# ekimb/rust-mdbg

Measured on AMD Instinct MI355X. Metric: Gbases/s ingested to k-min-mer graph, higher is better.
Workload: dtype u64

## Files before the change

### rust_mdbg_amd/csrc/context.inc

```
namespace {
struct KeptReads {
    void* blk = nullptr; size_t cap = 0; void* xblk = nullptr; size_t xcap = 0;
    u64 n_reads = 0, n_bases = 0, n_words = 0, n_exc = 0;
    KeptReads() = default; KeptReads(const KeptReads&) = delete; KeptReads& operator=(const KeptReads&) = delete;
    ~KeptReads() { if (blk) mdbg_block_free(blk, cap); if (xblk) mdbg_block_free(xblk, xcap); }
    uint2* planes() const { return (uint2*)blk; }
    u64* offsets() const { return (u64*)blk + n_words; }
    u64* exc_pos() const { return (u64*)xblk; }
    u8* exc_val() const { return (u8*)xblk + n_exc * 8; }
    u64 bytes() const { return n_words * 8 + (n_reads + 1) * 8 + n_exc * 9; }
};
struct Batch { u64 first_ordinal; u32 n_reads; u32 slot0; u64 m0, m1; u64 owned = ~0ull;
               u64 list_off = ~0ull;
               bool mread_ok = true;
               u32 src_rank = ~0u;
               u64 n_bases = 0;
               bool partial = false;
               u64 adm_word = ~0ull;
               std::shared_ptr<KeptReads> kept; };

enum { SH_DISTINCT = 0, SH_OWNED, SH_OWNINS, SH_FIN_WRAPPED, SH_FIN_DISTINCT, N_SHARD_ARRAYS };
enum { SC_CARRY = 0, SC_NDISTINCT, SC_NWINDOWS, SC_FIN0, SC_FIN1, SC_FIN2, SC_SLOWCOUNT , SC_ERRFLAG , SC_CAPERR , SC_SLOWTOTAL, SC_BATCHWIN, SC_IMPORTERR, SC_PROBEERR , SC_OWNINS, SC_OVERMAX , SC_TOTFIRST, SC_TOTSOLID, SC_SLICEFAIL, SC_DONE , SC_N };

}
// ... 5 lines not shown
    std::mutex err_mu;
    Stage stage[2]; std::mutex stage_mu; std::condition_variable stage_cv;
    mdbg_params P{};
    int dev = 0; hipStream_t stream = nullptr; std::string err; int poisoned = 0;
    u64 scal_seq = 0; bool batchwin_zero = false;
    u64* h_scal = nullptr;
    u64 bound = 0; DevBuf d_t4;
    DevBuf mh, mpos, mread, roff; u64 M = 0; u64 mcap = 0; u32 n_slots = 0;
    u64 slot_end_m = 0;
    u64 pending_m = 0;
    std::vector<Batch> batches; size_t batches_inserted = 0;
    u64 h_known = 0;
    DevBuf bread, tile_recs, slab, n_valid, n_scan, last_read, tile_base, scan_tmp, gran_sum, tile_flags, scalars, phase_dbg, shards;
    u32 slab_cap_min = 0;
    DevBuf tab, mx; u64 cap = 0;
    DevBuf pf_cells, pf_adm;
    u64 pf_n_cells = 0;
    size_t pf_counted = 0;
    bool pf_stale = false, pf_dirty = false;
    u64 n_windows_admitted = 0;
    DevBuf arena, route_out, route_tmp, route_h, route_f; u64 n_records = 0; bool routed = false;
    DevBuf by_maps;
    DevBuf link_ctr;
    DevBuf claim;
    bool claims_ok = false;
    size_t claims_fin_batches = 0; u64 claims_fin_top = 0;
    DevBuf bm_first, bm_solid, pre_first, pre_solid, popc_tmp, bt_dev, fin_out, solid_list, fin_order;
    DevBuf bm_local, pre_local, pre_local2;
    std::vector<u64> so_hash, so_pos, so_off;
    std::vector<u32> q_counts; std::vector<u64> q_off; DevBuf q_dev;
// ... 35 lines not shown
#define HIPCHK(c, call) do { hipError_t e_ = (call); if (e_ != hipSuccess) return fail_hip((c), #call, e_); } while (0)
#define MDBG_ENTER(c, args_ok) if (!(c) || !(args_ok)) return MDBG_E_PARAM; MDBG_LOCK(c); (void)hipSetDevice((c)->dev); if ((c)->poisoned) return fail((c), MDBG_E_STATE, "context is in an error state")
struct HandOver {
    mdbg_ctx* c; const char* what; bool to_host; int err = MDBG_OK;
    template <class T> void col(const T* dev, size_t n, HostRaw<T>& h, const T** dst) {
        if (err) return;
        if (!to_host) { *dst = dev; return; }
        if (!h.resize(n)) { err = fail(c, MDBG_E_NOMEM, what); return; }
        if (n) { const hipError_t e = hipMemcpy(h.data(), dev, n * sizeof(T), hipMemcpyDeviceToHost); if (e != hipSuccess) { err = fail_hip(c, what, e); return; } }
        *dst = h.data();
    }
};
bool nothing_resident(const mdbg_ctx* c) { return c->cap == 0 || c->M == 0; }

u64* scal(mdbg_ctx* c) { return c->scalars.as<u64>(); }
int read_scalars(mdbg_ctx* c, u64* host, bool with_fin = false, bool zero_batchwin = false) {
    if (!c->h_scal) { HIPCHK(c, hipHostMalloc((void**)&c->h_scal, (SC_N + 1) * 8, hipHostMallocMapped)); c->h_scal[SC_N] = 0; }
    const u64 seq = ++c->scal_seq;
    PublishArgs pa{};
    pa.shards[0] = c->shards.as<u64>() + SH_DISTINCT * CTR_SHARDS; pa.idx[0] = SC_NDISTINCT; pa.n_arrays = 1;
    pa.zero_mask = 0; pa.zero_arrays = 0;
    if (with_fin) {
        pa.shards[1] = c->shards.as<u64>() + SH_FIN_WRAPPED * CTR_SHARDS; pa.idx[1] = SC_FIN1; pa.shards[2] = c->shards.as<u64>() + SH_FIN_DISTINCT * CTR_SHARDS; pa.idx[2] = SC_FIN2; pa.n_arrays = 3;
        pa.zero_mask = (1ull << SC_FIN0) | (1ull << SC_FIN1) | (1ull << SC_FIN2); pa.zero_arrays = 0x6u;
    }
    pa.scalars = scal(c); pa.n = SC_N; pa.host = c->h_scal; pa.seq = seq; pa.zero_idx = zero_batchwin ? (u32)SC_BATCHWIN : (u32)SC_N;
    c->batchwin_zero = zero_batchwin;
    launch_publish_scalars(pa, c->stream);
    volatile u64* const flag = c->h_scal + SC_N;
    bool seen = false;
    const double t0 = now_ms();
    for (u32 spins = 0; !seen; ++spins) {
// ... 48 lines not shown
    const u64 mul = owner_bin_mul(c);
    if (!mul || c->batches.empty()) return MDBG_OK;
    Batch& b = which == ~(size_t)0 ? c->batches.back() : c->batches[which];
    fill_mread_of(c, b);
    launch_owner_bins(c->mh.as<u64>(), c->mread.as<u32>(), c->roff.as<u64>(), b.m0, b.m1, c->P.k, mul, d_hist, c->stream);
    return MDBG_OK;
}
int owner_set_table(mdbg_ctx* c, u32 world, const u8* tab) {
    const u64 mul = owner_bin_mul(c);
    if (!mul || !owner_thr(c, world)) return MDBG_OK;
    HIPCHK(c, hipMemcpyAsync(c->own_thr.as<u64>() + OWNER_TAB_AT, tab, OWNER_BINS, hipMemcpyHostToDevice, c->stream));
    HIPCHK(c, hipMemcpyAsync(c->own_thr.as<u64>(), &mul, 8, hipMemcpyHostToDevice, c->stream));
    HIPCHK(c, hipStreamSynchronize(c->stream));
    return MDBG_OK;
}
TableArgs table_args(mdbg_ctx* c) {
    TableArgs T;
    T.tab = c->tab.as<Slot>(); T.cap = c->cap; T.mx = c->mx.as<u64>(); T.A = cascade_of(c->P.min_abundance);
    T.n_distinct = c->shards.as<u64>() + SH_DISTINCT * CTR_SHARDS;
    T.ks.mh = c->mh.as<u64>(); T.ks.arena = c->arena.as<u64>(); T.ks.k = c->P.k;
    T.own_world = c->own_world; T.own_rank = c->own_rank; T.own_thr = owner_thr(c, c->own_world);
    T.probe_err = (u32*)(scal(c) + SC_PROBEERR); T.own_inserted = c->shards.as<u64>() + SH_OWNINS * CTR_SHARDS;
    T.claim = (!c->routed && c->claims_ok) ? c->claim.as<u8>() : nullptr;
    static const bool no_chain = getenv("MDBG_NO_CHAIN") != nullptr;
    T.no_chain = no_chain ? 1u : 0u;
    static const bool weak_fp = getenv("MDBG_WEAK_FP") != nullptr;
    T.fp_mask = weak_fp ? 0x3ull : 0x3FFFFFFFull;
    static const bool count_links = getenv("MDBG_COUNT_LINKS") != nullptr;
    T.link_ctr = nullptr;
    if (count_links) {
        if (!c->link_ctr.p && c->link_ctr.ensure(8, 0, c->stream) == hipSuccess) (void)hipMemsetAsync(c->link_ctr.p, 0, 8, c->stream);
// ... 7 lines not shown
int table_reserve(mdbg_ctx* c, u64 incoming) {
    u64 need = slots_for(c->n_distinct + incoming);
    const u32 A = cascade_of(c->P.min_abundance);
    if (c->cap == 0) {
        u64 want = need;
        if (c->P.table_capacity_hint) want = std::max(want, slots_for(c->P.table_capacity_hint));
        HIPCHK(c, c->tab.ensure(want * sizeof(Slot), 0, c->stream));
        if (A > 2) HIPCHK(c, c->mx.ensure(want * (A - 2) * 8, 0, c->stream));
        c->cap = want;
        launch_clear_table(c->tab.as<Slot>(), c->cap, c->mx.as<u64>(), A > 2 ? c->cap * (A - 2) : 0, c->stream);
        c->claims_ok = !c->routed && c->claim.p != nullptr;
        c->claims_fin_batches = 0;
        return MDBG_OK;
    }
    if (need <= c->cap) return MDBG_OK;
    need = std::max(need, 2 * c->cap);
    DevBuf ntab, nmx;
    HIPCHK(c, ntab.ensure(need * sizeof(Slot), 0, c->stream));
    if (A > 2) HIPCHK(c, nmx.ensure(need * (A - 2) * 8, 0, c->stream));
    launch_clear_table(ntab.as<Slot>(), need, nmx.as<u64>(), A > 2 ? need * (A - 2) : 0, c->stream);
    TableArgs T = table_args(c);
    T.tab = ntab.as<Slot>(); T.cap = need; T.mx = nmx.as<u64>();
    launch_rehash(c->tab.as<Slot>(), c->cap, c->mx.as<u64>(), T, c->stream);
    HIPCHK(c, hipStreamSynchronize(c->stream));
    std::swap(c->tab.p, ntab.p); std::swap(c->tab.cap, ntab.cap);
    std::swap(c->mx.p, nmx.p); std::swap(c->mx.cap, nmx.cap);
    c->cap = need;
    return MDBG_OK;
}

int clear_table(mdbg_ctx* c) {
    c->res.invalidate(FROM_NODES);
    ZeroList z{};
    z.p[0] = c->shards.as<u64>() + SH_DISTINCT * CTR_SHARDS; z.n[0] = CTR_SHARDS; z.p[1] = scal(c) + SC_NDISTINCT; z.n[1] = 2;
    z.p[2] = scal(c) + SC_IMPORTERR; z.n[2] = 1; z.p[3] = scal(c) + SC_PROBEERR; z.n[3] = 1;
    if (c->cap) launch_clear_table(c->tab.as<Slot>(), c->cap, c->mx.as<u64>(), cascade_of(c->P.min_abundance) > 2 ? c->cap * (cascade_of(c->P.min_abundance) - 2) : 0, c->stream, &z);
    else launch_zero_regions(z, c->stream);
    c->n_distinct = 0; c->n_windows = 0; c->n_windows_admitted = 0; c->batches_inserted = 0; c->n_records = 0; c->routed = false;
    c->claims_ok = c->claim.p != nullptr; c->claims_fin_batches = 0;
    return MDBG_OK;
}

#define STAGE_EVENT(c, ev, s) do { if ((c)->timing >= 2) HIPCHK((c), hipEventRecord((ev), (s))); } while (0)
hipEvent_t next_tile_event(mdbg_ctx* c) {
    if (c->timing < 1) return nullptr;
    if (c->tile_ev_used == c->tile_ev.size()) { hipEvent_t e = nullptr; if (hipEventCreate(&e) != hipSuccess) return nullptr; c->tile_ev.push_back(e); }
    return c->tile_ev[c->tile_ev_used++];
}
void collect_tile_events(mdbg_ctx* c) {
    for (size_t i = 0; i + 1 < c->tile_ev_used; i += 2) {
        float ms = 0;
// ... 110 lines not shown
```

### rust_mdbg_amd/csrc/dev_util.hip

```cpp
#include "mdbg_dev.h"
struct ZeroList { u64* p[6]; u64 n[6]; u64* set_p; u64 set_v; };
__global__ __launch_bounds__(256) void zero_regions_kernel(ZeroList z) {
    const u64 i0 = (u64)blockIdx.x * blockDim.x + threadIdx.x, stride = (u64)gridDim.x * blockDim.x;
#pragma unroll
    for (int r = 0; r < 6; ++r) for (u64 i = i0; i < z.n[r]; i += stride) z.p[r][i] = 0;
    if (i0 == 0 && z.set_p) *z.set_p = z.set_v;
}
void launch_zero_regions(const ZeroList& z, hipStream_t s) {
    u64 mx = 1;
    for (int r = 0; r < 6; ++r) mx = z.n[r] > mx ? z.n[r] : mx;
    const unsigned blocks = (unsigned)std::min<u64>(1024, (mx + 255) / 256);
    hipLaunchKernelGGL(zero_regions_kernel, dim3(blocks), dim3(256), 0, s, z);
}
__global__ __launch_bounds__(256) void fill_u64_kernel(u64* __restrict__ p, u64 n, u64 v) {
    for (u64 i = (u64)blockIdx.x * blockDim.x + threadIdx.x; i < n; i += (u64)gridDim.x * blockDim.x) p[i] = v;
}
void launch_fill_u64(u64* p, u64 n, u64 v, hipStream_t s) {
    if (n) hipLaunchKernelGGL(fill_u64_kernel, dim3((unsigned)std::min<u64>(1024, (n + 255) / 256)), dim3(256), 0, s, p, n, v);
}

__global__ __launch_bounds__(256) void sum_shards_kernel(const u64* __restrict__ shards, u64* __restrict__ out) {
    __shared__ u64 ws[4];
    const u64* s = shards + (size_t)blockIdx.x * CTR_SHARDS;
    u64 v = 0;
// ... 66 lines not shown
```

### rust_mdbg_amd/csrc/finalize_api.inc

```
static int fin_setup(mdbg_ctx* c, FinArgs& F, u64& n_words_out, bool byte_maps = false) {
    hipStream_t s = c->stream;
    c->res.invalidate(FROM_NODES);
    F.ath_override = nullptr;
    const u32 k = c->P.k;
        std::vector<Batch> bs = c->batches;
        std::sort(bs.begin(), bs.end(), [](const Batch& a, const Batch& b) { return a.first_ordinal < b.first_ordinal; });
        const u32 nb = (u32)bs.size();
        for (u32 i = 0; i + 1 < nb; ++i)
            if (bs[i].n_reads && bs[i].first_ordinal + bs[i].n_reads > bs[i + 1].first_ordinal) {
                char buf[200]; snprintf(buf, sizeof buf, "read ordinals of two batches overlap: [%llu, +%u) and [%llu, +%u) (first_read_ordinal must be the position of the batch's first record in the whole input)",
                                        (unsigned long long)bs[i].first_ordinal, bs[i].n_reads, (unsigned long long)bs[i + 1].first_ordinal, bs[i + 1].n_reads);
                return fail(c, MDBG_E_PARAM, buf);
            }
        std::vector<u64> fo(nb), rb(nb); std::vector<u32> nr(nb), s0(nb);
        u64 acc = 0;
        for (u32 i = 0; i < nb; ++i) { fo[i] = bs[i].first_ordinal; nr[i] = bs[i].n_reads; s0[i] = bs[i].slot0; rb[i] = acc; acc += bs[i].m1 - bs[i].m0; }
        std::vector<Batch> bs2 = c->batches;
        std::sort(bs2.begin(), bs2.end(), [](const Batch& a, const Batch& b) { return a.slot0 < b.slot0; });
        std::vector<u64> f2(nb), m2(nb), r2(nb); std::vector<u32> s2(nb);
        for (u32 i = 0; i < nb; ++i) { f2[i] = bs2[i].first_ordinal; s2[i] = bs2[i].slot0; }
        {
            std::vector<u32> ord(nb);
            for (u32 i = 0; i < nb; ++i) ord[i] = i;
            std::sort(ord.begin(), ord.end(), [&](u32 a, u32 b) { return bs[a].m0 != bs[b].m0 ? bs[a].m0 < bs[b].m0 : bs[a].m1 < bs[b].m1; });
// ... 279 lines not shown
```

### rust_mdbg_amd/csrc/import_api.inc

```
int mdbg_set_partition(mdbg_ctx* c, uint32_t world, uint32_t rank) {
    if (!c) return MDBG_E_PARAM;
    MDBG_LOCK(c);
    if (world < 1 || world > 4096 || rank >= world) return fail(c, MDBG_E_PARAM, "bad partition");
    if (world > 1 && prefilter_on(c)) return fail(c, MDBG_E_STATE, PF_UNAVAILABLE);
    if (c->n_distinct || c->batches_inserted) return fail(c, MDBG_E_STATE, "set the partition before inserting");
    c->own_world = world; c->own_rank = rank;
    return MDBG_OK;
}

int mdbg_sketch_view(mdbg_ctx* c, mdbg_sketch_store* out) {
    if (!c || !out) return MDBG_E_PARAM;
    MDBG_LOCK(c);
    (void)hipSetDevice(c->dev);
    HIPCHK(c, hipStreamSynchronize(c->stream));
    out->n_minimizers = c->M; out->n_reads = c->n_slots;
    out->d_hashes = c->mh.as<u64>(); out->d_positions = c->mpos.as<u32>(); out->d_read_offsets = c->roff.as<u64>();
    return MDBG_OK;
}

int mdbg_ingest_sketch(mdbg_ctx* c, const uint64_t* d_hashes, const uint32_t* d_positions, const uint64_t* d_read_offsets, uint64_t n_reads,
                       uint64_t first_read_ordinal) {
    if (!c) return MDBG_E_PARAM;
    MDBG_LOCK(c);
    (void)hipSetDevice(c->dev);
// ... 48 lines not shown
}

static int sketch_commit_impl(mdbg_ctx* c, uint64_t region, uint64_t n_minimizers, const uint64_t* d_read_offsets, uint64_t n_reads, uint64_t first_read_ordinal,
                              uint64_t owned_windows, bool with_read_map) {
    MDBG_LOCK(c);
    (void)hipSetDevice(c->dev);
    if (c->poisoned) return fail(c, MDBG_E_STATE, "context is in an error state");
    if (n_minimizers > c->pending_m || region + n_minimizers > c->M) return fail(c, MDBG_E_PARAM, "not a reserved region");
    if (n_reads && !d_read_offsets) return fail(c, MDBG_E_PARAM, "null offsets");
    if (first_read_ordinal + n_reads >= (1ull << (64 - WIN_BITS))) return fail(c, MDBG_E_CAPACITY, "read ordinal too large");
    store_commit_region(c, n_minimizers);
    if (!n_reads) return MDBG_OK;
    hipStream_t s = c->stream;
    u32 slot0 = 0;
    { int e = next_slot0(c, region, n_reads, &slot0); if (e) return e; }
    launch_rebase_offsets_checked(d_read_offsets, (u32)n_reads, region, n_minimizers, c->roff.as<u64>() + slot0, scal(c) + SC_IMPORTERR, s);
    if (with_read_map) launch_fill_mread(c->roff.as<u64>(), slot0, (u32)n_reads, c->mread.as<u32>(), s);
    Batch b; b.first_ordinal = first_read_ordinal; b.n_reads = (u32)n_reads; b.slot0 = slot0; b.m0 = region; b.m1 = region + n_minimizers;
    b.owned = owned_windows; b.mread_ok = with_read_map;
    store_append(c, b);
    return MDBG_OK;
}
int mdbg_sketch_commit(mdbg_ctx* c, uint64_t region, uint64_t n_minimizers, const uint64_t* d_read_offsets, uint64_t n_reads, uint64_t first_read_ordinal,
                       uint64_t owned_windows) {
    if (!c) return MDBG_E_PARAM;
    return sketch_commit_impl(c, region, n_minimizers, d_read_offsets, n_reads, first_read_ordinal, owned_windows, true);
}

int mdbg_owner_counts(mdbg_ctx* c, uint32_t world, uint64_t* counts) {
    if (!c || !counts) return MDBG_E_PARAM;
// ... 136 lines not shown
```

### rust_mdbg_amd/csrc/ingest_api.inc

```
namespace {
constexpr u64 SLAB_BUDGET = 6ull << 30;
int insert_resident_impl(mdbg_ctx* c, bool allow_pending = false);

constexpr const char* TABLE_FULL = "the table filled up during insertion";
int close_round(mdbg_ctx* c, const u64* sc, const char* probe_msg, float ms) {
    if ((u32)sc[SC_PROBEERR]) return fail(c, MDBG_E_PARAM, probe_msg);
    c->ms_insert += ms;
    c->n_windows += sc[SC_BATCHWIN];
    c->n_distinct = sc[SC_NDISTINCT];
    if (sc[SC_IMPORTERR]) return fail(c, MDBG_E_PARAM, "read offsets of an imported sketch are not consistent with its size");
    if ((u32)sc[SC_CAPERR]) return fail(c, MDBG_E_CAPACITY, "a read has more than 2^26 minimizers");
    return MDBG_OK;
}

struct SketchCall {
    const SketchInput& in; const u64* d_offsets; u64 n_reads, n_bases, first_ordinal, n_tiles_total; u32 slot0; bool phase_dbg;
};
int check_sketch_call(mdbg_ctx* c, const SketchInput& in, const u64* d_offsets, u64 n_reads, u64 n_bases, u64 first_ordinal, u64 n_tiles_total) {
    if (in.fmt == FMT_ASCII && !in.d_bases && n_bases) return fail(c, MDBG_E_PARAM, "null bases");
    if (in.fmt == FMT_PLANES && !in.d_planes && n_bases) return fail(c, MDBG_E_PARAM, "null packed words");
    if (!d_offsets) return fail(c, MDBG_E_PARAM, "null offsets");
    if ((((uintptr_t)in.d_bases) | ((uintptr_t)in.d_planes)) & 15) return fail(c, MDBG_E_PARAM, "device bases pointer must be 16-byte aligned");
    if (in.n_exc && (!in.d_exc_pos || !in.d_exc_val)) return fail(c, MDBG_E_PARAM, "null exception list");
    if (in.n_exc >= 0xFFFFFFF0ull) return fail(c, MDBG_E_CAPACITY, "too many exceptions");
// ... 46 lines not shown
    (void)hipStreamSynchronize(s);
    (void)hipMemcpy(h.data(), A.dbg, h.size() * 8, hipMemcpyDeviceToHost);
    double ph[7] = {0, 0, 0, 0, 0, 0, 0}, nc = 0, nv = 0; u64 nfast = 0;
    for (u32 t = 0; t < A.n_tiles; ++t) {
        const u64* q = &h[(size_t)t * 16];
        if (!q[7]) continue;
        ++nfast;
        ph[0] += (double)(q[1] - q[0]); ph[1] += (double)(q[2] - q[1]); ph[2] += (double)(q[3] - q[2]); ph[3] += (double)(q[4] - q[3]);
        ph[4] += (double)(q[5] - q[4]); ph[5] += (double)(q[7] - q[5]);
        nc += (double)q[9]; nv += (double)q[10];
    }
    const double n = nfast ? (double)nfast : 1.0;
    fprintf(stderr, "[mdbg phase timing] tiles=%u fast=%llu avg cycles: load=%.0f compact=%.0f hash=%.0f exact=%.0f rank=%.0f write=%.0f ; candidates=%.1f valid=%.1f slab_cap=%u\n",
            A.n_tiles, (unsigned long long)nfast, ph[0] / n, ph[1] / n, ph[2] / n, ph[3] / n, ph[4] / n, ph[5] / n, nc / n, nv / n, slab_cap);
}
int launch_tiles(mdbg_ctx* c, const SketchCall& k, SketchArgs& A, SketchInit init0, const TileParts& tp, const SlabPlan& sp) {
    hipStream_t s = c->stream;
    const SketchInput& in = k.in;
    A.bread = c->bread.as<u32>(); A.recs = c->tile_recs.as<TileRec>(); A.n_tiles = (u32)k.n_tiles_total;
    A.slab = c->slab.as<Rec>(); A.slab_cap = sp.slab_cap; A.n_valid = c->n_valid.as<u32>(); A.n_scan = c->n_scan.as<u32>(); A.last_read = c->last_read.as<u32>(); A.over_max = (u32*)(scal(c) + SC_OVERMAX);
    A.t4 = c->d_t4.as<u64>();
    A.tile_flags = in.n_exc ? c->tile_flags.as<u8>() : nullptr;
    A.err_flag = (u32*)(scal(c) + SC_ERRFLAG); A.slow_total = (unsigned long long*)(scal(c) + SC_SLOWTOTAL);
    A.read_base = k.slot0; A.bound = c->bound; A.btop = (u32)(c->bound >> (64 - BS_B)); A.force_slow = ((c->P.flags & 1u) || c->P.l > (u32)BS_MAX_L) ? 1u : 0u;
    A.dbg = nullptr;
    { const char* sp_ = getenv("MDBG_STOP_PHASE"); A.stop_phase = sp_ ? (u32)atoi(sp_) : 0u; }
    if (k.phase_dbg) { HIPCHK(c, c->phase_dbg.ensure((size_t)k.n_tiles_total * 128, 0, s)); HIPCHK(c, hipMemsetAsync(c->phase_dbg.p, 0, (size_t)k.n_tiles_total * 128, s)); A.dbg = c->phase_dbg.as<u64>(); }
    const u32 n_gran = (u32)((tp.max_part + SCAN_GRAN - 1) / SCAN_GRAN);
    HIPCHK(c, c->gran_sum.ensure((size_t)n_gran * 8 + 64, 0, s));
    A.block_sum = (unsigned long long*)c->gran_sum.as<u64>();
    init0.zero_arr = c->gran_sum.as<u64>(); init0.zero_arr_n = n_gran;
// ... 2 lines not shown
        HIPCHK(c, hipMemsetAsync(c->tile_flags.p, 0, k.n_tiles_total, s));
        launch_tile_flags(in.d_exc_pos, (u32)in.n_exc, A.n_tiles, c->tile_flags.as<u8>(), s);
    }
    if (c->P.scheme == MDBG_SCHEME_SYNCMERS) {
        A.scheme = 1; A.s = c->P.syncmer_s; A.btop = 0;
        const double v = c->P.density * (double)(1ull << (2 * c->P.l));
        A.bound = !(v > 0.0) ? 0 : (v >= 18446744073709551616.0 ? ~0ull : (u64)v);
        A.force_slow = ((c->P.flags & 1u) || c->P.syncmer_s > 13) ? 1u : 0u;
    }
    u64 t0 = 0;
    for (size_t pi = 0; pi < tp.part_end.size(); ++pi) {
        const u32 nt = (u32)(tp.part_end[pi] - t0);
        Rec* const part_slab = c->slab.as<Rec>();
        A.tile0 = (u32)t0; A.slab = part_slab;
        if (pi) HIPCHK(c, hipMemsetAsync(c->gran_sum.p, 0, (size_t)n_gran * 8, s));
        { hipEvent_t tb = next_tile_event(c), te = next_tile_event(c); launch_sketch(A, nt, s, tb, te); }
        GatherArgs G = gather_args(c, k, (u32)t0, nt, part_slab, sp.slab_cap, A.n_valid, pi + 1 == tp.part_end.size(), sp.gather_tiles);
        G.n_scan = A.n_scan; G.last_read = A.last_read;
        launch_gather(G, c->scan_tmp.as<u64>(), c->tile_base.as<u64>(), scal(c) + SC_CARRY, s, c->gran_sum.as<u64>());
        c->n_tile_launches += 1;
        t0 = tp.part_end[pi];
    }
    c->n_tile_bases += k.n_bases;
    if (k.phase_dbg) dump_phase_timing(A, sp.slab_cap, s);
    return MDBG_OK;
}
int alphabet_rule_pass(mdbg_ctx* c, const SketchArgs& A, u64 first_ordinal) {
    hipStream_t s = c->stream;
    u64 which = ~0ull;
    HIPCHK(c, hipMemcpyAsync(scal(c) + SC_SLOWTOTAL, &which, 8, hipMemcpyHostToDevice, s));
    launch_alphabet_rule(A, (unsigned long long*)(scal(c) + SC_SLOWTOTAL), s);
// ... 17 lines not shown
    L.mh = c->mh.as<u64>(); L.mpos = c->mpos.as<u32>(); L.mread = c->mread.as<u32>(); L.m0 = c->M; L.m1 = m_new;
    L.offsets = k.d_offsets; L.slot0 = k.slot0; L.l = c->P.l; L.hpc = c->P.reads_already_hpc == 0 ? 1u : 0u;
    L.slab = c->slab.as<Rec>(); L.n_valid = c->n_valid.as<u32>();
    launch_lmer_filter(L, in.fmt, in.d_bases, in.d_planes, in.d_exc_pos, in.d_exc_val, (u32)in.n_exc, s);
    HIPCHK(c, hipMemcpyAsync(scal(c) + SC_CARRY, init, 8, hipMemcpyHostToDevice, s));
    const GatherArgs G = gather_args(c, k, 0, nb, L.slab, 256, L.n_valid, true, 1);
    launch_gather(G, c->scan_tmp.as<u64>(), c->tile_base.as<u64>(), scal(c) + SC_CARRY, s);
    u64 sc[SC_N];
    int e = read_scalars(c, sc); if (e) return e;
    m_new = sc[SC_CARRY];
    return MDBG_OK;
}
int launch_fused_insert(mdbg_ctx* c, const SketchCall& k) {
    hipStream_t s = c->stream;
    u32* const ins_flags = (u32*)(scal(c) + SC_CAPERR);
    launch_count_reserve(c->roff.as<u64>(), k.slot0, (u32)k.n_reads, c->P.k, scal(c) + SC_BATCHWIN, (u32*)(scal(c) + SC_DONE), c->shards.as<u64>() + SH_DISTINCT * CTR_SHARDS, scal(c) + SC_NDISTINCT,
                         c->cap, ins_flags + 1, scal(c) + SC_CARRY, c->mcap, (const u32*)(scal(c) + SC_OVERMAX), s);
    if (!c->ev3) HIPCHK(c, hipEventCreate(&c->ev3));
    launch_insert_windows(table_args(c), c->mh.as<u64>(), c->mread.as<u32>(), c->roff.as<u64>(), c->M, c->mcap, k.slot0, k.first_ordinal, scal(c) + SC_NWINDOWS, ins_flags, s, scal(c) + SC_CARRY);
    STAGE_EVENT(c, c->ev3, s);
    return MDBG_OK;
}
int fused_tail(mdbg_ctx* c, const u64* sc, bool* inserted) {
    c->res.invalidate(FROM_NODES);
    if (sc[SC_CAPERR] >> 32) return MDBG_OK;
    c->batches_inserted = c->batches.size();
    *inserted = true;
    float ms = 0;
    if (c->timing >= 2 && hipEventElapsedTime(&ms, c->ev1, c->ev3) != hipSuccess) { (void)hipGetLastError(); ms = 0; }
    return close_round(c, sc, TABLE_FULL, ms);
// ... 29 lines not shown
        init0.zero[0] = scal(c) + SC_ERRFLAG; init0.zero[1] = scal(c) + SC_SLOWTOTAL; init0.zero[2] = scal(c) + SC_OVERMAX; init0.set_p = scal(c) + SC_CARRY; init0.set_v = c->M;
        const bool fused = then_insert && inserted && n_tiles_total && tp.part_end.size() == 1 && !phase_dbg && c->cap && c->own_world <= 1 && !c->lmer_on && !c->routed && !c->pending_m && !prefilter_on(c) &&
                           c->batches_inserted == c->batches.size() && c->mcap > c->M && c->mcap - c->M <= 2 * (want - c->M) + (1u << 20) &&
                           want - c->M <= (48ull << 20);
        if (fused) init0.zero[3] = scal(c) + SC_BATCHWIN;
        if (!n_tiles_total) {
            ZeroList z{};
            z.p[0] = init0.zero[0]; z.n[0] = 1; z.p[1] = init0.zero[1]; z.n[1] = 1; z.p[2] = init0.zero[2]; z.n[2] = 1; z.set_p = init0.set_p; z.set_v = init0.set_v;
            launch_zero_regions(z, s);
            launch_fill_u64(c->roff.as<u64>() + slot0, n_reads + 1, c->M, s);
        }
        SketchArgs A{};
        A.bases = in.d_bases; A.planes = in.d_planes; A.fmt = in.fmt; A.n_bases = n_bases; A.offsets = d_offsets; A.n_reads = (u32)n_reads;
        A.exc_pos = in.d_exc_pos; A.exc_val = in.d_exc_val; A.n_exc = (u32)in.n_exc;
        A.l = c->P.l; A.hpc = c->P.reads_already_hpc == 0 ? 1u : 0u;
        if (n_tiles_total) { int e = launch_tiles(c, k, A, init0, tp, sp); if (e) return e; }
        STAGE_EVENT(c, c->ev1, s);
        if (fused) { int e = launch_fused_insert(c, k); if (e) return e; }
        u64 sc[SC_N];
        int e = read_scalars(c, sc, false, true); if (e) return e;
        c->ms_sketch += ev_ms(c);
        collect_tile_events(c);
        u64 m_new = sc[SC_CARRY];
        const u32 over = (u32)sc[SC_OVERMAX];
        if (over || m_new > c->mcap) {
            if (over) { sp.slab_cap = std::min<u32>((u32)tile_bases, (over + over / 8 + 15u) & ~7u); c->slab_cap_min = sp.slab_cap; }
            if (m_new > c->mcap) want = m_new + 65536;
            c->n_tile_launches -= tp.part_end.size(); c->n_tile_bases -= n_tiles_total ? n_bases : 0;
            continue;
        }
        if (m_new >= 0xFFFFFFF0ull) return fail(c, MDBG_E_CAPACITY, "more than 2^32 minimizers resident on one device");
// ... 109 lines not shown
        if (listed(c, b))
            launch_insert_listed(table_args(c), c->mh.as<u64>(), c->mread.as<u32>(), c->roff.as<u64>(), b.m0, b.m1, list_of(b), seg_of(b), b.owned, b.slot0, b.n_reads, b.first_ordinal, flags, s);
        else
            launch_insert_windows(table_args(c), c->mh.as<u64>(), c->mread.as<u32>(), c->roff.as<u64>(), b.m0, b.m1, b.slot0, b.first_ordinal,
                                  scal(c) + SC_NWINDOWS, flags, s, nullptr, 0, adm_of(c, b), b.m0);
    }
    return MDBG_OK;
}

int insert_round_impl(mdbg_ctx* c, bool allow_pending) {
    if (c->poisoned) return fail(c, MDBG_E_STATE, "context is in an error state");
    if (c->routed) return fail(c, MDBG_E_STATE, "table holds routed records; local insertion is not allowed");
    if (c->pending_m && !allow_pending) return fail(c, MDBG_E_STATE, "reserved sketch regions have not been committed");
    hipStream_t s = c->stream;
    const size_t first = c->batches_inserted, last = c->batches.size();
    c->res.invalidate(FROM_NODES);
    bool any = false;
    for (size_t i = first; i < last; ++i) any = any || c->batches[i].m1 > c->batches[i].m0;
    c->batches_inserted = last;
    if (!any) return MDBG_OK;
    u64 sc[SC_N];
    bool counts_known = c->own_world > 1;
    u64 known = 0;
    for (size_t i = first; i < last; ++i) { const Batch& b = c->batches[i]; if (b.m1 == b.m0) continue; if (b.owned == ~0ull) counts_known = false; else known += b.owned; }
    int e = prefilter_on(c) ? prefilter_admit(c, first, last) : count_round_windows(c, first, last, counts_known, known); if (e) return e;
    u32* const flags = (u32*)(scal(c) + SC_CAPERR);
    u64 total_idx = 0;
    for (size_t i = first; i < last; ++i) total_idx += c->batches[i].m1 - c->batches[i].m0;
    u64 slice = 32ull << 20;
    { const char* sv = getenv("MDBG_INSERT_SLICE"); if (sv) { const u64 v = strtoull(sv, nullptr, 10); if (v) slice = std::max<u64>(v, (u64)OWN_SPAN); } }
// ... 394 lines not shown
```

### rust_mdbg_amd/csrc/mdbg_dev.h

```cpp
#pragma once
#include <hip/hip_runtime.h>
#include <stdint.h>

typedef uint8_t u8;
typedef uint16_t u16;
typedef uint32_t u32;
typedef uint64_t u64;

constexpr int TILE_WPT = 4;
constexpr int TILE_THREADS = 256;
constexpr int TILE_RAW_WORDS = TILE_WPT * TILE_THREADS;
constexpr int TILE_HALO = 256;
constexpr int TILE_STRIDE = TILE_RAW_WORDS * 32 - TILE_HALO;
constexpr int MDBG_MAX_L_DEV = 32;

constexpr u32 MDBG_CASCADE_MAX = 8;
__host__ __device__ inline u32 cascade_of(u32 A) { return A <= MDBG_CASCADE_MAX ? A : 1u; }

constexpr int WIN_BITS = 26;
constexpr u64 WIN_MASK = (1ull << WIN_BITS) - 1;

struct __attribute__((aligned(16))) Rec {
    u64 hash;
    u32 pos;
    u32 read;
};

#define NT_SEED_A 0x3c8bfbb395c60474ull
#define NT_SEED_C 0x3193c18562a02b4cull
#define NT_SEED_G 0x20323ed082572324ull
#define NT_SEED_T 0x295549f54be24456ull

__host__ __device__ inline u64 rol64(u64 x, unsigned r) { r &= 63; return (x << r) | (x >> ((64 - r) & 63)); }

__device__ inline u64 nt_h_ascii(u8 c) {
// ... 51 lines not shown
```

### rust_mdbg_amd/csrc/sketch.hip

```cpp
#include "mdbg_dev.h"
#include "bs_core.h"

enum { FMT_ASCII = 0, FMT_PLANES = 1 };
constexpr int SCAN_GRAN_LOG = 6, SCAN_GRAN = 1 << SCAN_GRAN_LOG;
struct TileRec;

struct SketchArgs {
    const u8* bases;
    const uint2* planes;
    u32 fmt;
    u64 n_bases;
    const u64* offsets; u32 n_reads;
    const u32* bread;
    const TileRec* recs;
    u32 n_tiles;
    u32 tile0, tile_end;
    Rec* slab; u32 slab_cap;
    u32* n_valid;
    u32* n_scan;
    u32* last_read;
    u32* over_max;
    unsigned long long* block_sum;
    const u64* t4;
    const u8* tile_flags;
    const u64* exc_pos; const u8* exc_val; u32 n_exc;
    u32* err_flag; unsigned long long* slow_total;
    u32 read_base;
    u64 bound; u32 l; u32 hpc; u32 btop;
    u32 scheme, s;
    u32 force_slow;
    u64* dbg;
    u32 stop_phase;
};

__device__ inline u32 find_read(const u64* __restrict__ off, u32 lo, u32 hi, u64 p) {
    while (lo < hi) { u32 mid = lo + ((hi - lo + 1) >> 1); if (off[mid] <= p) lo = mid; else hi = mid - 1; }
    return lo;
}


constexpr int TREC_N = 7;
struct __attribute__((aligned(16))) TileRec { u32 rl, rh; int64_t start0; int32_t rel[TREC_N - 1]; int64_t first_base; };
static_assert(sizeof(TileRec) == 48, "three 16-byte words");
struct SketchInit { u64* zero[4]; u64* set_p; u64 set_v; u64* zero_arr; u32 zero_arr_n; };
__global__ void tile_rec_kernel(const u64* __restrict__ off, u32 n_reads, u64 n_bases, u32 n_tiles, u32* __restrict__ bread, TileRec* __restrict__ recs, SketchInit init,
                                int64_t stride, int64_t halo) {
    const u32 t = blockIdx.x * blockDim.x + threadIdx.x;
// ... 319 lines not shown
    };
    run(false, 0);
    if (n_mine > SYNC_KEEP) any_over = 1;
    u32 total;
    const u32 base = block_excl_scan_256(n_mine, sc_tmp, total);
    if (!any_over) {
        for (u32 i = 0; i < n_mine; ++i) if (base + i < a.slab_cap) slab[base + i] = keep[i];
    } else run(true, base);
    if (tid == 0) put_count(a, gt, total);
}


struct CandOut { u64 hash; u32 pos, read; };

#define MDBG_HOT(cond, value) (cond)
template <int L, int SCHEME = 0, int WMAX = 1>
__global__ __launch_bounds__(TILE_THREADS, SCHEME ? 5 : 6) void sketch_bs_kernel(SketchArgs a) {
    constexpr int TT = TILE_THREADS, RW = TILE_RAW_WORDS, HW = TILE_HW, QCAP = TILE_QCAP, RS_CAP = TILE_RS_CAP, STAGE_AT = TILE_STAGE_AT;
    __shared__ TileLdsS<SCHEME> S;
    __shared__ __attribute__((aligned(16))) u64 S_t3[T3_WORDS];
    __shared__ u32 sync_tmp[SCHEME ? 16 : 1];
    const u32 Lr = SCHEME ? a.l : (u32)L;
    const int tid = (int)threadIdx.x, lane = tid & 63, wv = tid >> 6;
    const int64_t nb = (int64_t)a.n_bases;
    const int64_t n_pairs = (nb + 31) >> 5;
    const bool hpc = MDBG_HOT(a.hpc != 0, true);
    typedef u32 u32x4 __attribute__((ext_vector_type(4)));
    const u32 wg = blockIdx.x, gt = a.tile0 + wg;
    Rec* const slab = a.slab + (size_t)wg * a.slab_cap;
#define MDBG_STAMP(i) do { if (a.dbg && tid == 0) a.dbg[(size_t)gt * 16 + (i)] = __builtin_readcyclecounter(); } while (0)
// ... 15 lines not shown
            const u32x4* src = (const u32x4*)(a.bases + raw0);
#pragma unroll
            for (int g = 0; g < CPT; ++g) { const u32x4 q = __builtin_nontemporal_load(src + tid + TT * g); av[g] = make_uint4(q.x, q.y, q.z, q.w); }
        }
    } else {
        if (interior) {
            const u32x4* src = (const u32x4*)(a.planes + pi0);
#pragma unroll
            for (int i = 0; i < WPT / 2; ++i) { const u32x4 q = __builtin_nontemporal_load(src + i); pr[2 * i] = make_uint2(q.x, q.y); pr[2 * i + 1] = make_uint2(q.z, q.w); }
        } else {
#pragma unroll
            for (int i = 0; i < WPT; ++i) { const int64_t pi = pi0 + i; pr[i] = (pi >= 0 && pi < n_pairs) ? a.planes[pi] : make_uint2(0u, 0u); }
        }
        if (tid && pi0 - 1 >= 0 && pi0 - 1 < n_pairs) { const uint2 q = a.planes[pi0 - 1]; pv0 = q.x >> 31; pv1 = q.y >> 31; }
    }
    const u32 rl = (u32)__builtin_amdgcn_readfirstlane((int)rec->rl), rh_ = (u32)__builtin_amdgcn_readfirstlane((int)rec->rh);
    static_assert((2 * (DPAD + RW + 4)) % 4 == 0, "the dense stream is a whole number of 16-byte words");
    for (int i = tid; i < 2 * (DPAD + RW + 4) / 4; i += TT) ((uint4*)S.dense)[i] = make_uint4(0u, 0u, 0u, 0u);
    if (SCHEME == 0) {
        static_assert(T3_WORDS % 128 == 0, "the table is copied 16 bytes per lane");
        for (int i = tid; i < T3_WORDS / 2; i += TT) ((uint4*)S_t3)[i] = ((const uint4*)a.t4)[i];
    } else {
        u32 v = 0;
        for (int i = 0; i < 8; ++i) v |= ((u32)tid >> i & 1u) << (2 * i);
        ((u16*)S_t3)[tid] = (u16)v;
    }
    if (tid == 0) { S.misc[8] = a.force_slow | ((a.tile_flags && a.tile_flags[gt]) ? 1u : 0u); S.misc[9] = 0; S.misc[11] = 0; S.misc[17] = 0; S.misc[18] = 0; S.misc[19] = 0; S.misc[20] = 0; }
    __syncthreads();
    if (MDBG_HOT(rh_ - rl < (u32)TREC_N, true)) {
        if ((u32)tid <= rh_ - rl) {
// ... 1007 lines not shown
```

Before: 2603.

## Defer hash-table clear and fuse it into the sketch tile kernel

Resetting the table no longer launches a separate clear kernel. It marks a clear as pending, and the first sketch launch of a fused ingest spreads the table and overflow-word fill across its workgroups. The fill runs while those workgroups wait on their base loads, so the pass over the table can overlap with sketch work instead of running as its own kernel. Every other path that touches the table flushes a pending clear eagerly first. The cost is extra stores in the sketch kernel, a per-tile size cap, and added correctness risk if any consumer misses the flush.

```diff
diff --git a/rust_mdbg_amd/csrc/context.inc b/rust_mdbg_amd/csrc/context.inc
--- a/rust_mdbg_amd/csrc/context.inc
+++ b/rust_mdbg_amd/csrc/context.inc
@@ -43,6 +43,7 @@
     DevBuf bread, tile_recs, slab, n_valid, n_scan, last_read, tile_base, scan_tmp, gran_sum, tile_flags, scalars, phase_dbg, shards;
     u32 slab_cap_min = 0;
     DevBuf tab, mx; u64 cap = 0;
+    bool clear_pending = false; ZeroList clear_z{};
     DevBuf pf_cells, pf_adm;
     u64 pf_n_cells = 0;
     size_t pf_counted = 0;
@@ -108,8 +109,10 @@
 bool nothing_resident(const mdbg_ctx* c) { return c->cap == 0 || c->M == 0; }
 
 u64* scal(mdbg_ctx* c) { return c->scalars.as<u64>(); }
+void table_flush_clear(mdbg_ctx* c);
 int read_scalars(mdbg_ctx* c, u64* host, bool with_fin = false, bool zero_batchwin = false) {
     if (!c->h_scal) { HIPCHK(c, hipHostMalloc((void**)&c->h_scal, (SC_N + 1) * 8, hipHostMallocMapped)); c->h_scal[SC_N] = 0; }
+    table_flush_clear(c);
     const u64 seq = ++c->scal_seq;
     PublishArgs pa{};
     pa.shards[0] = c->shards.as<u64>() + SH_DISTINCT * CTR_SHARDS; pa.idx[0] = SC_NDISTINCT; pa.n_arrays = 1;
@@ -188,7 +191,34 @@
     HIPCHK(c, hipStreamSynchronize(c->stream));
     return MDBG_OK;
 }
+u64 mx_words(const mdbg_ctx* c, u64 cap) { const u32 A = cascade_of(c->P.min_abundance); return A > 2 ? cap * (A - 2) : 0; }
+void table_flush_clear(mdbg_ctx* c) {
+    if (!c->clear_pending) return;
+    c->clear_pending = false;
+    launch_clear_table(c->tab.as<Slot>(), c->cap, c->mx.as<u64>(), mx_words(c, c->cap), c->stream, &c->clear_z);
+}
+bool eager_clear() { static const bool on = getenv("MDBG_EAGER_CLEAR") != nullptr; return on; }
+constexpr u64 FILL_MAX_BYTES_PER_TILE = 64ull << 10;
+constexpr u64 FILL_CARRIER_BYTES = 32ull << 10;
+u64 fill_max_bytes_per_tile() { static const u64 v = getenv("MDBG_FILL_MAX_KB") ? strtoull(getenv("MDBG_FILL_MAX_KB"), nullptr, 10) << 10 : FILL_MAX_BYTES_PER_TILE; return v; }
+bool take_tile_fill(mdbg_ctx* c, u32 n_wg, TileFill& f) {
+    f = TileFill{};
+    if (!c->clear_pending || !c->cap || !n_wg || eager_clear()) return false;
+    const u64 n_mx = mx_words(c, c->cap);
+    if ((c->cap * sizeof(Slot) + n_mx * 8) / n_wg > fill_max_bytes_per_tile()) return false;
+    static_assert(sizeof(Slot) == 32, "two 16-byte words per slot");
+    const u64 share = (c->cap * sizeof(Slot) + n_mx * 8) / n_wg;
+    while (f.carrier_log < 6 && (share << (f.carrier_log + 1)) <= FILL_CARRIER_BYTES) ++f.carrier_log;
+    const u32 n_carriers = (u32)(((u64)n_wg + (1u << f.carrier_log) - 1) >> f.carrier_log);
+    f.tab = (uint4*)c->tab.p; f.n_tab = 2 * c->cap; f.per_tab = fill_words_per_wg(f.n_tab, n_carriers);
+    f.mx = (uint4*)c->mx.p; f.n_mx = n_mx / 2; f.per_mx = fill_words_per_wg(f.n_mx, n_carriers);
+    f.mx_tail = (n_mx & 1) ? c->mx.as<u64>() + (n_mx - 1) : nullptr;
+    f.z = c->clear_z; f.on = 1;
+    c->clear_pending = false;
+    return true;
+}
 TableArgs table_args(mdbg_ctx* c) {
+    table_flush_clear(c);
     TableArgs T;
     T.tab = c->tab.as<Slot>(); T.cap = c->cap; T.mx = c->mx.as<u64>(); T.A = cascade_of(c->P.min_abundance);
     T.n_distinct = c->shards.as<u64>() + SH_DISTINCT * CTR_SHARDS;
@@ -226,6 +256,7 @@
         return MDBG_OK;
     }
     if (need <= c->cap) return MDBG_OK;
+    table_flush_clear(c);
     need = std::max(need, 2 * c->cap);
     DevBuf ntab, nmx;
     HIPCHK(c, ntab.ensure(need * sizeof(Slot), 0, c->stream));
@@ -246,7 +277,7 @@
     ZeroList z{};
     z.p[0] = c->shards.as<u64>() + SH_DISTINCT * CTR_SHARDS; z.n[0] = CTR_SHARDS; z.p[1] = scal(c) + SC_NDISTINCT; z.n[1] = 2;
     z.p[2] = scal(c) + SC_IMPORTERR; z.n[2] = 1; z.p[3] = scal(c) + SC_PROBEERR; z.n[3] = 1;
-    if (c->cap) launch_clear_table(c->tab.as<Slot>(), c->cap, c->mx.as<u64>(), cascade_of(c->P.min_abundance) > 2 ? c->cap * (cascade_of(c->P.min_abundance) - 2) : 0, c->stream, &z);
+    if (c->cap) { c->clear_pending = true; c->clear_z = z; }
     else launch_zero_regions(z, c->stream);
     c->n_distinct = 0; c->n_windows = 0; c->n_windows_admitted = 0; c->batches_inserted = 0; c->n_records = 0; c->routed = false;
     c->claims_ok = c->claim.p != nullptr; c->claims_fin_batches = 0;
diff --git a/rust_mdbg_amd/csrc/dev_util.hip b/rust_mdbg_amd/csrc/dev_util.hip
--- a/rust_mdbg_amd/csrc/dev_util.hip
+++ b/rust_mdbg_amd/csrc/dev_util.hip
@@ -1,5 +1,4 @@
 #include "mdbg_dev.h"
-struct ZeroList { u64* p[6]; u64 n[6]; u64* set_p; u64 set_v; };
 __global__ __launch_bounds__(256) void zero_regions_kernel(ZeroList z) {
     const u64 i0 = (u64)blockIdx.x * blockDim.x + threadIdx.x, stride = (u64)gridDim.x * blockDim.x;
 #pragma unroll
diff --git a/rust_mdbg_amd/csrc/finalize_api.inc b/rust_mdbg_amd/csrc/finalize_api.inc
--- a/rust_mdbg_amd/csrc/finalize_api.inc
+++ b/rust_mdbg_amd/csrc/finalize_api.inc
@@ -1,5 +1,6 @@
 static int fin_setup(mdbg_ctx* c, FinArgs& F, u64& n_words_out, bool byte_maps = false) {
     hipStream_t s = c->stream;
+    table_flush_clear(c);
     c->res.invalidate(FROM_NODES);
     F.ath_override = nullptr;
     const u32 k = c->P.k;
diff --git a/rust_mdbg_amd/csrc/import_api.inc b/rust_mdbg_amd/csrc/import_api.inc
--- a/rust_mdbg_amd/csrc/import_api.inc
+++ b/rust_mdbg_amd/csrc/import_api.inc
@@ -86,6 +86,7 @@
     hipStream_t s = c->stream;
     u32 slot0 = 0;
     { int e = next_slot0(c, region, n_reads, &slot0); if (e) return e; }
+    table_flush_clear(c);
     launch_rebase_offsets_checked(d_read_offsets, (u32)n_reads, region, n_minimizers, c->roff.as<u64>() + slot0, scal(c) + SC_IMPORTERR, s);
     if (with_read_map) launch_fill_mread(c->roff.as<u64>(), slot0, (u32)n_reads, c->mread.as<u32>(), s);
     Batch b; b.first_ordinal = first_read_ordinal; b.n_reads = (u32)n_reads; b.slot0 = slot0; b.m0 = region; b.m1 = region + n_minimizers;
diff --git a/rust_mdbg_amd/csrc/ingest_api.inc b/rust_mdbg_amd/csrc/ingest_api.inc
--- a/rust_mdbg_amd/csrc/ingest_api.inc
+++ b/rust_mdbg_amd/csrc/ingest_api.inc
@@ -84,7 +84,7 @@
     fprintf(stderr, "[mdbg phase timing] tiles=%u fast=%llu avg cycles: load=%.0f compact=%.0f hash=%.0f exact=%.0f rank=%.0f write=%.0f ; candidates=%.1f valid=%.1f slab_cap=%u\n",
             A.n_tiles, (unsigned long long)nfast, ph[0] / n, ph[1] / n, ph[2] / n, ph[3] / n, ph[4] / n, ph[5] / n, nc / n, nv / n, slab_cap);
 }
-int launch_tiles(mdbg_ctx* c, const SketchCall& k, SketchArgs& A, SketchInit init0, const TileParts& tp, const SlabPlan& sp) {
+int launch_tiles(mdbg_ctx* c, const SketchCall& k, SketchArgs& A, SketchInit init0, const TileParts& tp, const SlabPlan& sp, bool carry_fill) {
     hipStream_t s = c->stream;
     const SketchInput& in = k.in;
     A.bread = c->bread.as<u32>(); A.recs = c->tile_recs.as<TileRec>(); A.n_tiles = (u32)k.n_tiles_total;
@@ -117,7 +117,9 @@
         Rec* const part_slab = c->slab.as<Rec>();
         A.tile0 = (u32)t0; A.slab = part_slab;
         if (pi) HIPCHK(c, hipMemsetAsync(c->gran_sum.p, 0, (size_t)n_gran * 8, s));
+        if (carry_fill && pi == 0) (void)take_tile_fill(c, nt, A.fill);
         { hipEvent_t tb = next_tile_event(c), te = next_tile_event(c); launch_sketch(A, nt, s, tb, te); }
+        A.fill = TileFill{};
         GatherArgs G = gather_args(c, k, (u32)t0, nt, part_slab, sp.slab_cap, A.n_valid, pi + 1 == tp.part_end.size(), sp.gather_tiles);
         G.n_scan = A.n_scan; G.last_read = A.last_read;
         launch_gather(G, c->scan_tmp.as<u64>(), c->tile_base.as<u64>(), scal(c) + SC_CARRY, s, c->gran_sum.as<u64>());
@@ -165,6 +167,7 @@
 int launch_fused_insert(mdbg_ctx* c, const SketchCall& k) {
     hipStream_t s = c->stream;
     u32* const ins_flags = (u32*)(scal(c) + SC_CAPERR);
+    table_flush_clear(c);
     launch_count_reserve(c->roff.as<u64>(), k.slot0, (u32)k.n_reads, c->P.k, scal(c) + SC_BATCHWIN, (u32*)(scal(c) + SC_DONE), c->shards.as<u64>() + SH_DISTINCT * CTR_SHARDS, scal(c) + SC_NDISTINCT,
                          c->cap, ins_flags + 1, scal(c) + SC_CARRY, c->mcap, (const u32*)(scal(c) + SC_OVERMAX), s);
     if (!c->ev3) HIPCHK(c, hipEventCreate(&c->ev3));
@@ -224,7 +227,7 @@
         A.bases = in.d_bases; A.planes = in.d_planes; A.fmt = in.fmt; A.n_bases = n_bases; A.offsets = d_offsets; A.n_reads = (u32)n_reads;
         A.exc_pos = in.d_exc_pos; A.exc_val = in.d_exc_val; A.n_exc = (u32)in.n_exc;
         A.l = c->P.l; A.hpc = c->P.reads_already_hpc == 0 ? 1u : 0u;
-        if (n_tiles_total) { int e = launch_tiles(c, k, A, init0, tp, sp); if (e) return e; }
+        if (n_tiles_total) { int e = launch_tiles(c, k, A, init0, tp, sp, fused); if (e) return e; }
         STAGE_EVENT(c, c->ev1, s);
         if (fused) { int e = launch_fused_insert(c, k); if (e) return e; }
         u64 sc[SC_N];
@@ -364,6 +367,7 @@
     if (c->pending_m && !allow_pending) return fail(c, MDBG_E_STATE, "reserved sketch regions have not been committed");
     hipStream_t s = c->stream;
     const size_t first = c->batches_inserted, last = c->batches.size();
+    table_flush_clear(c);
     c->res.invalidate(FROM_NODES);
     bool any = false;
     for (size_t i = first; i < last; ++i) any = any || c->batches[i].m1 > c->batches[i].m0;
diff --git a/rust_mdbg_amd/csrc/mdbg_dev.h b/rust_mdbg_amd/csrc/mdbg_dev.h
--- a/rust_mdbg_amd/csrc/mdbg_dev.h
+++ b/rust_mdbg_amd/csrc/mdbg_dev.h
@@ -19,6 +19,8 @@
 
 constexpr int WIN_BITS = 26;
 constexpr u64 WIN_MASK = (1ull << WIN_BITS) - 1;
+
+struct ZeroList { u64* p[6]; u64 n[6]; u64* set_p; u64 set_v; };
 
 struct __attribute__((aligned(16))) Rec {
     u64 hash;
diff --git a/rust_mdbg_amd/csrc/sketch.hip b/rust_mdbg_amd/csrc/sketch.hip
--- a/rust_mdbg_amd/csrc/sketch.hip
+++ b/rust_mdbg_amd/csrc/sketch.hip
@@ -1,9 +1,19 @@
 #include "mdbg_dev.h"
 #include "bs_core.h"
+#include "table_fill.h"
 
 enum { FMT_ASCII = 0, FMT_PLANES = 1 };
 constexpr int SCAN_GRAN_LOG = 6, SCAN_GRAN = 1 << SCAN_GRAN_LOG;
 struct TileRec;
+
+struct TileFill {
+    uint4* tab; u64 n_tab, per_tab;
+    uint4* mx; u64 n_mx, per_mx;
+    u64* mx_tail;
+    ZeroList z;
+    u32 on;
+    u32 carrier_log;
+};
 
 struct SketchArgs {
     const u8* bases;
@@ -31,6 +41,7 @@
     u32 force_slow;
     u64* dbg;
     u32 stop_phase;
+    TileFill fill;
 };
 
 __device__ inline u32 find_read(const u64* __restrict__ off, u32 lo, u32 hi, u64 p) {
@@ -380,6 +391,21 @@
 struct CandOut { u64 hash; u32 pos, read; };
 
 #define MDBG_HOT(cond, value) (cond)
+__device__ __forceinline__ void tile_fill_region(uint4* __restrict__ base, u64 n, u64 per, u32 wg, int tid, const uint4 v) {
+    fill_lane_words(n, per, wg, (u32)tid, [&](u64 i) { base[i] = v; });
+}
+__device__ __forceinline__ void tile_fill(const TileFill& f, u32 wg, int tid) {
+    static_assert(FILL_GRAIN == TILE_THREADS, "one word per lane and trip");
+    const u32 ones = 0xFFFFFFFFu;
+    tile_fill_region(f.tab, f.n_tab, f.per_tab, wg, tid, (tid & 1) ? make_uint4(ones, ones, 0u, 0u) : make_uint4(ones, ones, ones, ones));
+    if (f.n_mx) tile_fill_region(f.mx, f.n_mx, f.per_mx, wg, tid, make_uint4(ones, ones, ones, ones));
+    if (wg == 0) {
+#pragma unroll
+        for (int r = 0; r < 6; ++r) for (u64 i = (u64)tid; i < f.z.n[r]; i += TILE_THREADS) f.z.p[r][i] = 0;
+        if (tid == 0 && f.z.set_p) *f.z.set_p = f.z.set_v;
+        if (tid == 0 && f.mx_tail) *f.mx_tail = ~0ull;
+    }
+}
 template <int L, int SCHEME = 0, int WMAX = 1>
 __global__ __launch_bounds__(TILE_THREADS, SCHEME ? 5 : 6) void sketch_bs_kernel(SketchArgs a) {
     constexpr int TT = TILE_THREADS, RW = TILE_RAW_WORDS, HW = TILE_HW, QCAP = TILE_QCAP, RS_CAP = TILE_RS_CAP, STAGE_AT = TILE_STAGE_AT;
@@ -425,6 +451,7 @@
         }
         if (tid && pi0 - 1 >= 0 && pi0 - 1 < n_pairs) { const uint2 q = a.planes[pi0 - 1]; pv0 = q.x >> 31; pv1 = q.y >> 31; }
     }
+    if (MDBG_HOT(a.fill.on != 0, true)) { if ((wg & ((1u << a.fill.carrier_log) - 1u)) == 0) tile_fill(a.fill, wg >> a.fill.carrier_log, tid); }
     const u32 rl = (u32)__builtin_amdgcn_readfirstlane((int)rec->rl), rh_ = (u32)__builtin_amdgcn_readfirstlane((int)rec->rh);
     static_assert((2 * (DPAD + RW + 4)) % 4 == 0, "the dense stream is a whole number of 16-byte words");
     for (int i = tid; i < 2 * (DPAD + RW + 4) / 4; i += TT) ((uint4*)S.dense)[i] = make_uint4(0u, 0u, 0u, 0u);
diff --git a/rust_mdbg_amd/csrc/table_fill.h b/rust_mdbg_amd/csrc/table_fill.h
--- /dev/null
+++ b/rust_mdbg_amd/csrc/table_fill.h
@@ -0,0 +1,28 @@
+#pragma once
+#include <stdint.h>
+#if defined(__HIPCC__)
+#define TF_HD __host__ __device__ __forceinline__
+#else
+#define TF_HD inline
+#endif
+
+constexpr uint64_t FILL_GRAIN = 256;
+
+TF_HD uint64_t fill_words_per_wg(uint64_t n, uint32_t n_wg) {
+    if (!n_wg) return 0;
+    const uint64_t per = n / n_wg + (n % n_wg ? 1 : 0);
+    return (per + FILL_GRAIN - 1) / FILL_GRAIN * FILL_GRAIN;
+}
+TF_HD void fill_slice(uint64_t n, uint64_t per, uint32_t wg, uint64_t& lo, uint64_t& hi) {
+    lo = per * wg;
+    if (lo > n) lo = n;
+    hi = n - lo < per ? n : lo + per;
+}
+template <class Store> TF_HD void fill_lane_words(uint64_t n, uint64_t per, uint32_t wg, uint32_t tid, Store&& store) {
+    uint64_t lo, hi;
+    fill_slice(n, per, wg, lo, hi);
+    const uint64_t cnt = hi - lo;
+    uint64_t i = lo + tid;
+    for (uint64_t j = cnt / FILL_GRAIN; j; --j, i += FILL_GRAIN) store(i);
+    if (tid < cnt % FILL_GRAIN) store(i);
+}
```

Result: slower. 2571 (-1.2%).
